# XuyangBai/PointDSC

Hardware: AMD Instinct MI355X
Metric: point-cloud pairs/sec @ N=5000 corr (higher is better)
Workload: dtype f32 (attention products as fp16x3 split (fp16 hi+lo operand pairs, three f16 MFMAs per product), f32 accumulate; fc_message / PointCN products as fp16 hi+lo split; spatial-consistency matrix stored as unorm16); 1 GPU; 3DMatch-like synthetic correspondences (BASELINE.json configs[2]): N=5000 corr, 32 pairs per step sharded over 1 GPU(s) = 32 per GPU, 12-layer PointDSC, seeded random weights; num_corr=5000, pairs_per_gpu=32, global_batch=32, compat_format=u16, layer_gemm=h3, att_leaves=canonical, latency_mode=False, range_guard=lazy (pipeline), collective=none (single process, no process group)

## Files before the change

include/pointdsc_hip.h:

```cpp
#ifndef POINTDSC_HIP_H
#define POINTDSC_HIP_H

#include <stddef.h>

#ifdef __cplusplus
extern "C" {
#endif

#define PDSC_VERSION 9
#define PDSC_CHANNELS 128
#define PDSC_MAX_K 64
#define PDSC_MAX_POWER_ITERS 32

enum pdsc_status {
    PDSC_OK = 0,
    PDSC_ERR_ARG = -1,
    PDSC_ERR_WORKSPACE = -2,
    PDSC_ERR_LAUNCH = -3
};

typedef struct pdsc_config {
    int in_dim;
    int num_layers;
    int num_channels;
// ... 145 lines not shown
int    pdsc_pack_qkv_split(const float* qkv, void* q_split, void* kv_tiles, int bs, int N, void* stream);
size_t pdsc_attention_split_scratch_bytes(int bs, int N, int nsplit);
int    pdsc_attention_split_default_split(int bs, int N);
int    pdsc_attention_leaf_count(int N);
int    pdsc_attention_leaf_plan(int bs, int N, int leaves_mode, int* nsplit, int* nleaf);
size_t pdsc_attention_leaf_scratch_bytes(int bs, int N, int leaves_mode);
int    pdsc_sc_attention_split(const void* q_split, const void* kv_tiles, const float* compat, long long ld,
                               float* msg, void* scratch, size_t scratch_bytes, int bs, int N, int nsplit,
                               void* stream);
int    pdsc_sc_attention_split_u16(const void* q_split, const void* kv_tiles, const unsigned short* compat_u16, long long ld,
                                   float* msg, void* scratch, size_t scratch_bytes, int bs, int N, int nsplit,
                                   void* stream);

int pdsc_attention_trace(long long* device_buffer);

int pdsc_layer_trace(long long* device_buffer);

int pdsc_classifier_hidden(const float* feat, const float* W1, const float* b1, const float* W2, const float* b2, float* h2,
                           int M, void* stream);

int pdsc_normalize_confidence(const float* feat, const float* h2, const float* w3, const float* b3,
                              float* normed, float* conf, int M, void* stream);

int pdsc_nms_keys(const float* src_keypts, const float* conf, float radius, float* keys,
                  int bs, int N, void* stream);
size_t pdsc_nms_workspace_bytes(int bs, int N);
int pdsc_nms_keys_grid(const float* src_keypts, const float* conf, float radius, float* keys, void* workspace,
                       size_t workspace_bytes, int bs, int N, void* stream);
int pdsc_rank_select(const float* keys, int* seeds, int bs, int N, int num_seeds, void* stream);

// ... 187 lines not shown
```

pointdsc_amd/_lib.py:

```python
from __future__ import annotations

import ctypes as C
import os
from pathlib import Path

PKG = Path(__file__).resolve().parent
LIB_PATH = Path(os.environ.get("POINTDSC_HIP_LIB", PKG / "libpointdsc_hip.so"))


class PointDSCLibraryError(RuntimeError):
    pass


class PdscConfig(C.Structure):
    _fields_ = [
        ("in_dim", C.c_int), ("num_layers", C.c_int), ("num_channels", C.c_int),
        ("num_iterations", C.c_int), ("k", C.c_int), ("refine_iters", C.c_int),
        ("inlier_threshold", C.c_float), ("nms_radius", C.c_float), ("refine_threshold", C.c_float),
        ("attention_precision", C.c_int), ("compat_format", C.c_int), ("layer_gemm", C.c_int),
        ("att_leaves", C.c_int), ("value_fold", C.c_int),
    ]


W_SECTIONS = [
# ... 40 lines not shown
    "pdsc_wfrag_head_bytes": (_sz, []),
    "pdsc_wfrag_fold_tail_bytes": (_sz, []),
    "pdsc_wfrag_fold_head_bytes": (_sz, []),
    "pdsc_wfrag_build_tail": (_i, [_vp] * 7 + [_i, _vp]),
    "pdsc_wfrag_build_head": (_i, [_vp] * 5 + [_i, _vp]),
    "pdsc_sc_attention_split_partials": (_i, [_vp, _vp, _vp, _i, _ll, _vp, _sz, _i, _i, _i, _i, _vp]),
    "pdsc_split_q_bytes": (_sz, [_i, _i]),
    "pdsc_split_kv_bytes": (_sz, [_i, _i]),
    "pdsc_pack_qkv_split": (_i, [_vp, _vp, _vp, _i, _i, _vp]),
    "pdsc_attention_split_scratch_bytes": (_sz, [_i, _i, _i]),
    "pdsc_attention_split_default_split": (_i, [_i, _i]),
    "pdsc_attention_leaf_count": (_i, [_i]),
    "pdsc_attention_leaf_plan": (_i, [_i, _i, _i, C.POINTER(C.c_int), C.POINTER(C.c_int)]),
    "pdsc_attention_leaf_scratch_bytes": (_sz, [_i, _i, _i]),
    "pdsc_attention_trace": (_i, [_vp]),
    "pdsc_layer_trace": (_i, [_vp]),
    "pdsc_sc_attention_split": (_i, [_vp, _vp, _vp, _ll, _vp, _vp, _sz, _i, _i, _i, _vp]),
    "pdsc_sc_attention_split_u16": (_i, [_vp, _vp, _vp, _ll, _vp, _vp, _sz, _i, _i, _i, _vp]),
    "pdsc_attention_scratch_bytes": (_sz, [_i, _i, _i]),
    "pdsc_attention_default_split": (_i, [_i, _i]),
    "pdsc_sc_attention": (_i, [_vp, _vp, _ll, _vp, _vp, _sz, _i, _i, _i, _vp]),
    "pdsc_normalize_confidence": (_i, [_vp, _vp, _vp, _vp, _vp, _vp, _i, _vp]),
    "pdsc_nms_keys": (_i, [_vp, _vp, _f, _vp, _i, _i, _vp]),
    "pdsc_nms_workspace_bytes": (_sz, [_i, _i]),
    "pdsc_nms_keys_grid": (_i, [_vp, _vp, _f, _vp, _vp, _sz, _i, _i, _vp]),
    "pdsc_rank_select": (_i, [_vp, _vp, _i, _i, _i, _vp]),
    "pdsc_knn_seeds": (_i, [_vp, _vp, _vp, _vp, _i, _i, _i, _i, _vp]),
    "pdsc_knn_seeds_form": (_i, [_vp, _vp, _vp, _vp, _vp, _i, _i, _i, _i, _i, _vp]),
    "pdsc_normalize_confidence_pf": (_i, [_vp, _vp, _vp, _vp, _vp, _vp, _vp, _i, _i, _vp]),
    "pdsc_seed_power_iteration": (_i, [_vp, _vp, _vp, _vp, _vp, _vp, _vp, _vp, _vp, _i, _i, _i, _i, _i, _vp]),
# ... 97 lines not shown
```

pointdsc_amd/csrc/api.hip:

```cpp
#include <stdarg.h>
#include <stdlib.h>
#include <string.h>
#include <mutex>
#include "pdsc_common.h"
#include "ragged.h"
#include "attention_common.h"
#include "layer_args.h"

namespace pdsc {

static thread_local char g_err[512] = "";

static unsigned int*& range_report_slot() {
    static thread_local unsigned int* slot = nullptr;
    return slot;
}

void set_error(const char* fmt, ...) {
    va_list ap;
    va_start(ap, fmt);
    vsnprintf(g_err, sizeof(g_err), fmt, ap);
    va_end(ap);
}

// ... 333 lines not shown
    do {                               \
        const int rc__ = (call);       \
        if (rc__ != PDSC_OK) return rc__; \
    } while (0)

struct EncoderPlan {
    bool fused;
    bool split;
    LayerKernel kernel;
    bool x3, frag;
    bool fuse_merge;
    bool pf, leaves, fold;
    int gemm;
    int ns, Npad;
    int nleaf, value_width;
    int ws_tail, ws_head;
};

static int plan_encoder(const pdsc_config* cfg, int bs, int N, const int* nvalid, int n_min, EncoderPlan* plan) {
    EncoderPlan& p = *plan = EncoderPlan{};
    p.split = cfg->attention_precision != PDSC_ATT_FP32;
    p.x3 = cfg->attention_precision == PDSC_ATT_FP16X3_ALL;
    p.fused = env_int("PDSC_FUSED_LAYERS", 1) != 0 && cfg->num_layers > 0;
    const bool canonical = cfg->att_leaves >= PDSC_LEAVES_CANONICAL;
    const int min_tiles = (n_min + 31) / 32;
    p.ns = p.split ? pdsc_attention_split_default_split(bs, N) : 0;
#define PDSC_REQUIRE_SHORTEST_PAIR(cond)                                                                                             \
    PDSC_REQUIRE(cond, "pdsc_forward_testing_ragged: the shortest pair (%d correspondences) has fewer 32-key tiles than the key split " \
                 "planned for bs=%d, N=%d (%d): batch pairs of more similar size", n_min, bs, N, p.ns)
    if (nvalid && p.split && !canonical) PDSC_REQUIRE_SHORTEST_PAIR(min_tiles >= p.ns);
// ... 5 lines not shown
    if (!p.fused || !p.split) {
        p.kernel = by_size(1, bs * N);
        return PDSC_OK;
    }
    p.Npad = (int)round_up(N, 256);
    p.gemm = env_int("PDSC_LAYER_GEMM", cfg->layer_gemm) == PDSC_LAYER_GEMM_H3 ? PDSC_LAYER_GEMM_H3 : PDSC_LAYER_GEMM_F32;
    const bool h3 = p.gemm == PDSC_LAYER_GEMM_H3;
    const LayerKernel natural = by_size(bs, N);
    p.frag = env_int("PDSC_LAYER_FRAG", 1) && !p.x3 && !force_block && (natural == LayerKernel::Wave || h3);
    p.kernel = p.x3     ? LayerKernel::X3
               : !p.frag ? natural
                         : h3 && env_int("PDSC_LAYER_H3_VARIANT", 1) != 0 ? LayerKernel::H3 : LayerKernel::Wave;
    p.fuse_merge = env_int("PDSC_FUSE_MERGE", 1) && p.ns > 1 && p.ns <= layer_merge_limit(p.kernel);
    const bool pf_ok = p.kernel == LayerKernel::H3 && env_int("PDSC_LAYER_PF", 1) != 0;
    int lf_ns = 0, lf_nw = 0;
    if (canonical) leaf_plan(bs, N, cfg->att_leaves, &lf_nw, &lf_ns, &p.nleaf);
    p.leaves = pf_ok && canonical && (!nvalid || min_tiles >= 2 * p.nleaf);
    if (nvalid && !p.leaves) PDSC_REQUIRE_SHORTEST_PAIR(min_tiles >= p.ns);
#undef PDSC_REQUIRE_SHORTEST_PAIR
    p.pf = p.leaves || (pf_ok && p.fuse_merge);
    p.fold = cfg->value_fold == PDSC_VALUE_FOLD_ON && p.pf && N <= PDSC_VALUE_FOLD_MAX_N;
    p.value_width = p.fold ? PDSC_CHANNELS / 2 : PDSC_CHANNELS;
    p.ws_tail = p.fold ? PDSC_WS_FOLD_TAIL_H3 : h3 ? PDSC_WS_FRAG_TAIL_H3 : PDSC_WS_FRAG_TAIL;
    p.ws_head = p.fold ? PDSC_WS_FOLD_HEAD_H3 : h3 ? PDSC_WS_FRAG_HEAD_H3 : PDSC_WS_FRAG_HEAD;
    return PDSC_OK;
}

enum class ForwardMode { Testing, Validation, Probe };

struct ForwardCall {
    ForwardMode mode;
// ... 86 lines not shown
    else
        PDSC_TRY(pdsc_spatial_compat(c.src, c.tgt, x.W(PDSC_W_SIGMA_SPAT, 0), x.compat, nullptr, x.ld, c.bs, c.N, x.st));
    PDSC_TRY(launch_layer0(c.corr_pos, c.cfg->in_dim, x.W(PDSC_W_LAYER0_W, 0), x.W(PDSC_W_LAYER0_B, 0), x.featA, x.M, x.range_flag, c.bs, x.st));
    return probe_absmax(x, PDSC_RANGE_LAYER0, x.featA, (size_t)x.M * PDSC_CHANNELS);
}

static int attention_split(const ForwardCtx& x, float* msg_out, int nsplit) {
    return launch_attention_split_ex(x.q_split, x.kv_tiles, x.compat, x.cfmt, x.ld, msg_out, x.att_scratch, x.L.bytes[WS_ATT_SCRATCH], x.c.bs,
                                     x.c.N, nsplit, PDSC_PARTIALS_ROWS, x.c.nvalid, x.st);
}

static int run_fused_layer(const ForwardCtx& x, int i, bool last, const float* cur, float* nxt) {
    const EncoderPlan& plan = x.plan;
    const bool tail = i >= 0, head = !last, split = x.split;
    const bool parts = plan.pf || plan.fuse_merge;
    const int nparts = plan.leaves ? plan.nleaf : plan.ns;
    const float* part_o = parts ? (const float*)x.att_scratch : nullptr;
    const float* part_ml = parts ? part_o + (size_t)x.c.bs * nparts * plan.Npad * plan.value_width : nullptr;
    pdsc_layer_call c{};
    c.bs = split ? x.c.bs : 1; c.N = split ? x.c.N : x.M;
    if (tail) {
        c.msg = parts ? nullptr : x.msg;
        c.part_o = part_o; c.part_ml = part_ml; c.nsplit = nparts; c.Npad = plan.Npad;
        c.res = cur;
    } else
        c.feat_in = x.featA;
    if (last) c.feat_out = x.featA;
    if (head) {
        c.featB_out = nxt; c.qkv_out = split ? nullptr : x.qkv;
        c.q_split = x.q_split; c.kv_tiles = x.kv_tiles;
    }
    if (plan.frag) {
        if (tail) c.wfrag_tail = x.WS(plan.ws_tail, i);
// ... 1 lines not shown
        c.gemm_format = plan.gemm;
    } else {
        auto mat = [&](int section, int l) { return plan.x3 ? x.WS(section, l) : (const void*)x.W(section, l); };
        if (tail) {
            c.w1 = mat(PDSC_W_FC1_W, i); c.b1 = x.W(PDSC_W_FC1_B, i); c.w2 = mat(PDSC_W_FC2_W, i); c.b2 = x.W(PDSC_W_FC2_B, i);
            c.w3 = mat(PDSC_W_FC3_W, i); c.b3 = x.W(PDSC_W_FC3_B, i);
        }
        if (head) {
            c.wp = mat(PDSC_W_PCN_W, i + 1); c.bp = x.W(PDSC_W_PCN_B, i + 1); c.wq = mat(PDSC_W_QKV_W, i + 1); c.bq = x.W(PDSC_W_QKV_B, i + 1);
            if (split) c.wq_split = x.WS(PDSC_W_QKV_W, i + 1);
        }
    }
    if (plan.pf) c.io_flags = (tail ? PDSC_IO_PARTIALS_PF | PDSC_IO_RES_PF : 0) | (head ? PDSC_IO_FEATB_PF : 0);
    LayerArgs a = layer_args_from_call(c);
    a.nvalid = split ? x.c.nvalid : nullptr;
    if (plan.pf) {
        a.value_fold = plan.fold;
        a.range_flag = x.range_flag;
    } else
        a.trace = pdsc_layer_trace_buffer();
    PDSC_TRY(validate_layer_args(a, plan.kernel, "pdsc_forward_testing(layer)"));
    return dispatch_layer(a, plan.kernel, x.st);
}

static int run_encoder_fused(const ForwardCtx& x) {
    const ForwardCall& c = x.c;
    const EncoderPlan& plan = x.plan;
    const size_t att_bytes = x.L.bytes[WS_ATT_SCRATCH];
    PDSC_TRY(run_fused_layer(x, -1, false, nullptr, x.featB));
    float *cur = x.featB, *nxt = x.featC;
// ... 190 lines not shown
```

pointdsc_amd/csrc/attention_split.hip:

```cpp
#include <stdlib.h>
#include <type_traits>
#include "attention_common.h"
#include "split_layout.h"
#include "ragged.h"

namespace pdsc {


template <int NW, int BYTES>
__device__ __forceinline__ void issue_linear(__amdgpu_buffer_rsrc_t rsrc, int src_off, unsigned char* dst, int wave, unsigned lane16) {
    constexpr int PIECES = BYTES / 1024;
    static_assert(BYTES % 1024 == 0, "tile parts are whole KiB");
#pragma unroll
    for (int u = 0; u < (PIECES + NW - 1) / NW; ++u) {
        const int i = wave + NW * u;
        if ((u + 1) * NW <= PIECES || i < PIECES)
            __builtin_amdgcn_raw_ptr_buffer_load_lds(rsrc, (lptr_t)(dst + i * 1024), 16, lane16, src_off + i * 1024, 0, 0);
    }
}
__device__ __forceinline__ f32x16 scale_acc(f32x16 o, float alpha) {
#pragma unroll
    for (int r = 0; r < 16; ++r) {
        float v = o[r];
        asm volatile("v_mul_f32 %0, %0, %1" : "+v"(v) : "v"(alpha));
// ... 138 lines not shown
        dma_k(kt0);
        if (kt0 + 1 < kt1) dma_k(kt0 + 1);
        dma_v(kt0);
        asm volatile("s_waitcnt vmcnt(0)" ::: "memory");
        __syncthreads();
        for (int kt = kt0; kt < kt1; ++kt) {
            const int st = (kt - kt0) & 1;
            asm volatile("s_waitcnt vmcnt(0)" ::: "memory");
            __syncthreads();
            if (kt + 1 < kt1) {
#pragma unroll
                for (int slot = NCS; slot < DMA_SLOTS; ++slot) dma_slot(kt, st, slot);
            }
        }
        asm volatile("s_waitcnt vmcnt(0)" ::: "memory");
        if (!(a.nsplit != 1 && a.part_frag)) __syncthreads();
        return;
    }

    f32x4 ccur[4], cnext[4];
    dma_k(kt0); dma_c(kt0);
    if (CREG) creg_load(kt0, ccur);
    if (kt0 + 1 < kt1) { dma_k(kt0 + 1); dma_c(kt0 + 1); }
    if (CREG) creg_load(kt0 + 1, cnext);
    dma_v(kt0);
    sp16x8 qh[8], ql[8];
    auto load_q = [&](int pair, int qblock) {
        const int qrow = min(qblock * (NW * 32) + wave * 32 + l31, N - 1);
        const sp16* qsrc = a.qs + ((size_t)pair * NS + qrow) * SPL_Q_LD + 8 * h;
#pragma unroll
        for (int j = 0; j < 8; ++j) {
// ... 28 lines not shown
        for (int c = 0; c < NC; ++c)
#pragma unroll
            for (int g = 0; g < 4; ++g)
                *reinterpret_cast<f32x4*>(base + pf_offset_floats(4 * c + g)) = f32x4{o[c][4 * g], o[c][4 * g + 1], o[c][4 * g + 2], o[c][4 * g + 3]};
        if (h == 0) {
            a.part_ml[(slot_prev + l31) * 2 + 0] = m_prev;
            a.part_ml[(slot_prev + l31) * 2 + 1] = l_prev;
        }
#pragma unroll
        for (int c = 0; c < NC; ++c)
#pragma unroll
            for (int r = 0; r < 16; ++r) o[c][r] = 0.f;
    };

    const int q0w = qb * (NW * 32) + wave * 32;
    auto leaf_store = [&](int lf, float m_st, float l_st) {
        const size_t slot = ((size_t)b * a.nleaf + lf) * a.Npad + q0w;
        float* base = a.part_o + slot * VW + lane * 4;
#pragma unroll
        for (int c = 0; c < NC; ++c)
#pragma unroll
            for (int g = 0; g < 4; ++g)
                *reinterpret_cast<f32x4*>(base + pf_offset_floats(4 * c + g)) = f32x4{o[c][4 * g], o[c][4 * g + 1], o[c][4 * g + 2], o[c][4 * g + 3]};
        if (h == 0) {
            a.part_ml[(slot + l31) * 2 + 0] = m_st;
            a.part_ml[(slot + l31) * 2 + 1] = l_st;
        }
    };
    int leaf_prev = 0;

    const int koff = l31 * 16 + 512 * h;
    const int voff = l31 * 16 + (VW * 16) * h;
    const int crow_off = (wave * 32 + l31) * CROW;
    const int csw = C16 ? (l31 >> 2) & 3 : ((wave * 32 + l31) >> 1) & 7;
    constexpr float C16_INV = 1.0f / 65535.0f;
    typedef float f32x2 __attribute__((ext_vector_type(2)));
    f32x2 c16_inv2 = {C16_INV, C16_INV};
    asm volatile("" : "+v"(c16_inv2));
    auto c16_group = [&](const unsigned (&w)[8], int g, float (&cc)[4]) {
        const unsigned w0 = w[2 * g], w1 = w[2 * g + 1];
        const f32x2 a = f32x2{(float)(w0 & 0xffffu), (float)(w0 >> 16)} * c16_inv2;
        const f32x2 b = f32x2{(float)(w1 & 0xffffu), (float)(w1 >> 16)} * c16_inv2;
// ... 286 lines not shown
        b = b_n; sp = sp_n; qb = qb_n;
        kt0 = kt0n;
        kt1 = kt0 + per + (sp < rem ? 1 : 0);
        q_rows = q_rows_n;
        dK = 2; dV = 1;
        load_q(b, qb);
        l_run = 0.f;
        look_ahead();
    }
  }
    asm volatile("s_waitcnt vmcnt(0)" ::: "memory");
    if constexpr (PS) return;
    const float l_tot = l_run + __shfl_xor(l_run, 32, 64);
    const int q0 = qb * (NW * 32) + wave * 32;
    if constexpr (MG) {
        leaf_store(leaf, m_run, l_tot);
        return;
    }
    if (a.nsplit != 1 && a.part_frag) {
        float* base = a.part_o + (((size_t)b * a.nsplit + sp) * a.Npad + q0) * VW + lane * 4;
#pragma unroll
        for (int c = 0; c < NC; ++c)
#pragma unroll
            for (int g = 0; g < 4; ++g)
                *reinterpret_cast<f32x4*>(base + pf_offset_floats(4 * c + g)) = f32x4{o[c][4 * g], o[c][4 * g + 1], o[c][4 * g + 2], o[c][4 * g + 3]};
        if (h == 0 && q0 + l31 < a.Npad) {
            const size_t slot = ((size_t)b * a.nsplit + sp) * a.Npad + q0 + l31;
            a.part_ml[slot * 2 + 0] = m_run;
            a.part_ml[slot * 2 + 1] = l_tot;
        }
        if (TRACE) {
// ... 115 lines not shown
        const int rounds = ceil_div(wgs, slots);
        double cost = (double)rounds * (ceil_div(tiles, ns) + (ns > 1 ? 4.0 : 3.0));
        if (((ns * bs) & 7) != 0) cost *= 1.03;
        if (cost < best_cost - 1e-9) { best_cost = cost; best = ns; }
    }
    const int force_nw = env_int("PDSC_ATT_SPLIT_NW", 0), force_ns = env_int("PDSC_ATT_SPLIT_NS", 0);
    *nw_out = (force_nw == 4 || force_nw == 8) ? force_nw : nw;
    *nsplit_out = force_ns > 0 ? (force_ns < tiles ? force_ns : tiles) : best;
}

int attention_leaf_count(int N) {
    const int t = spl_num_tiles(N);
    return t >= 48 ? 4 : t >= 32 ? 8 : t >= 16 ? 4 : t >= 8 ? 2 : 1;
}

void leaf_plan(int bs, int N, int leaves_mode, int* nw_out, int* nsplit_out, int* nleaf_out) {
    int nw, ns;
    split_plan(bs, N, &nw, &ns);
    const int tiles = spl_num_tiles(N);
    int C = leaves_mode == PDSC_LEAVES_CANONICAL ? attention_leaf_count(N) : leaves_mode;
    if (C > tiles / 2) C = tiles / 2;
    if (C > PDSC_ATT_MAX_LEAVES) C = PDSC_ATT_MAX_LEAVES;
    if (C < 1) C = 1;
    const int nq = ceil_div(N, nw * 32), slots = nw == 8 ? 256 : 512;
    int best = 1;
    double best_cost = 1e30;
    for (int d = 1; d <= C; ++d) {
        if (C % d) continue;
        const int wgs = nq * bs * d, rounds = ceil_div(wgs, slots);
        double cost = (double)rounds * (ceil_div(tiles, d) + 4.0 + 0.35 * (C / d));
        if (((d * bs) & 7) != 0) cost *= 1.03;
        if (cost < best_cost - 1e-9) { best_cost = cost; best = d; }
    }
    *nw_out = nw; *nsplit_out = best; *nleaf_out = C;
}

}

using namespace pdsc;

extern "C" int pdsc_attention_leaf_count(int N) { return N > 0 ? attention_leaf_count(N) : -1; }

extern "C" int pdsc_attention_leaf_plan(int bs, int N, int leaves_mode, int* nsplit, int* nleaf) {
    PDSC_REQUIRE(bs > 0 && N > 0 && leaves_mode >= PDSC_LEAVES_CANONICAL && leaves_mode <= PDSC_ATT_MAX_LEAVES && nsplit && nleaf,
                 "pdsc_attention_leaf_plan: bs=%d N=%d leaves_mode=%d", bs, N, leaves_mode);
    int nw;
    leaf_plan(bs, N, leaves_mode, &nw, nsplit, nleaf);
    return PDSC_OK;
}

extern "C" size_t pdsc_attention_leaf_scratch_bytes(int bs, int N, int leaves_mode) {
    if (bs <= 0 || N <= 0 || leaves_mode < PDSC_LEAVES_CANONICAL) return 0;
    int nw, ns, C;
    leaf_plan(bs, N, leaves_mode, &nw, &ns, &C);
    return (size_t)bs * C * round_up(N, 256) * (PDSC_CHANNELS + 2) * sizeof(float);
}

int pdsc::launch_attention_leaves(const void* q_split, const void* kv_tiles, const void* compat, int compat_format, long long ld,
                                  void* scratch, size_t scratch_bytes, int bs, int N, int leaves_mode, const int* nvalid, int n_min,
                                  hipStream_t st, int value_width) {
    PDSC_REQUIRE(q_split && kv_tiles && compat && scratch, "pdsc_sc_attention_leaves: null pointer");
    PDSC_REQUIRE(value_width == PDSC_CHANNELS || value_width == PDSC_CHANNELS / 2, "pdsc_sc_attention_leaves: value_width=%d", value_width);
    const bool v64 = value_width != PDSC_CHANNELS;
    PDSC_REQUIRE(bs > 0 && N > 0, "pdsc_sc_attention_leaves: bs=%d N=%d", bs, N);
    PDSC_REQUIRE(compat_format == PDSC_COMPAT_F32 || compat_format == PDSC_COMPAT_U16, "pdsc_sc_attention_leaves: compat_format=%d", compat_format);
    const bool c16 = compat_format == PDSC_COMPAT_U16;
    PDSC_REQUIRE(ld >= round_up(N, SPL_BK) && ld % (c16 ? 8 : 4) == 0,
                 "pdsc_sc_attention_leaves: ld=%lld must be a multiple of %d and >= N rounded up to 32", ld, c16 ? 8 : 4);
    int nw, ns, C;
    leaf_plan(bs, N, leaves_mode, &nw, &ns, &C);
    PDSC_REQUIRE(!nvalid || (n_min + 31) / 32 >= 2 * C, "pdsc_sc_attention_leaves: the shortest pair (%d correspondences) has fewer than two "
                 "32-key tiles for each of the %d leaves planned for bs=%d, N=%d", n_min, C, bs, N);
    const size_t need = (size_t)bs * C * round_up(N, 256) * (value_width + 2) * sizeof(float);
    if (scratch_bytes < need) {
        set_error("pdsc_sc_attention_leaves: scratch %zu < %zu bytes", scratch_bytes, need);
        return PDSC_ERR_WORKSPACE;
    }
    const int tiles = spl_num_tiles(N);
    AttSplitArgs a{};
    a.qs = (const sp16*)q_split; a.kv = (const unsigned char*)kv_tiles; a.compat = compat; a.ld = ld; a.msg = nullptr;
    a.N = N; a.Npad = (int)round_up(N, 256); a.nsplit = ns; a.num_tiles = tiles; a.bs = bs;
    a.nq = ceil_div(N, nw * 32);
    a.nleaf = C;
    a.part_o = (float*)scratch;
    a.part_ml = a.part_o + (size_t)bs * C * a.Npad * value_width;
// ... 222 lines not shown
```

pointdsc_amd/csrc/layer.hip:

```cpp
#include <stdlib.h>
#include <type_traits>
#include "pdsc_common.h"
#include "split_layout.h"
#include "merge_partials.h"
#include "layer_args.h"
#include "layer_block.h"

namespace pdsc {

constexpr int LF_ROWS = 32;
constexpr int LF_LD = PDSC_CHANNELS + 4;
constexpr int LF_TILE = LF_ROWS * LF_LD;


#define LF_STAMP(k)                                                                                   \
    if (a.trace && lane == 0) a.trace[(((size_t)blockIdx.y * gridDim.x + blockIdx.x) * 4 + wave) * 16 + (k)] = __builtin_readcyclecounter();

template <int K>
__device__ __forceinline__ void load_w(const float* __restrict__ W, int n0, int l31, int h, f32x4 (&w)[K / 8]) {
    const float* p = W + (size_t)(n0 + l31) * K + 4 * h;
#pragma unroll
    for (int q = 0; q < K / 8; ++q) w[q] = *reinterpret_cast<const f32x4*>(p + 8 * q);
}

// ... 276 lines not shown
    const bool frag = h3 || (kernel == LayerKernel::Wave && (a.wf_tail || a.wf_head));
    const int io = a.io_flags;
    PDSC_REQUIRE(tail || head, "%s: neither tail (msg / partials) nor head (featB_out) requested", who);
    PDSC_REQUIRE(a.bs > 0 && a.N > 0, "%s: bs=%d N=%d", who, a.bs, a.N);
    PDSC_REQUIRE(a.gemm_format == PDSC_LAYER_GEMM_F32 || a.gemm_format == PDSC_LAYER_GEMM_H3, "%s: gemm_format=%d", who, a.gemm_format);
    PDSC_REQUIRE((io & ~(PDSC_IO_PARTIALS_PF | PDSC_IO_RES_PF | PDSC_IO_FEATB_PF)) == 0, "%s: io_flags=%d", who, io);
    PDSC_REQUIRE(h3 || (io == 0 && !a.value_fold), "%s: point-fragment hand-offs and the folded layer exist in the H3 kernel only", who);
    PDSC_REQUIRE(!h3 || a.gemm_format == PDSC_LAYER_GEMM_H3, "%s: point-fragment hand-offs need gemm_format = PDSC_LAYER_GEMM_H3", who);
    PDSC_REQUIRE(!a.value_fold || (io & PDSC_IO_PARTIALS_PF) || !tail, "%s: the folded layer merges point-fragment partials", who);
    if (tail) {
        PDSC_REQUIRE(a.res && (frag ? a.wf_tail != nullptr : a.w1 && a.b1 && a.w2 && a.b2 && a.w3 && a.b3),
                     "%s: tail needs res and fc1..fc3 (natural layout or the tail stream)", who);
        if (!a.msg) PDSC_REQUIRE(a.part_ml && a.nsplit >= 1 && a.nsplit <= layer_merge_limit(kernel) && a.Npad >= a.N,
                                 "%s: partials need part_ml, 1 <= nsplit <= %d (what this launch's kernel merges), Npad >= N", who,
                                 layer_merge_limit(kernel));
        PDSC_REQUIRE(!(io & PDSC_IO_PARTIALS_PF) || (!a.msg && a.Npad % 32 == 0), "%s: PF partials come un-merged (msg NULL), Npad a multiple of 32", who);
    } else {
        PDSC_REQUIRE(a.feat_in, "%s: head-only needs feat_in", who);
        PDSC_REQUIRE(!(io & (PDSC_IO_PARTIALS_PF | PDSC_IO_RES_PF)), "%s: head-only takes feat_in in row order", who);
    }
    if (head) PDSC_REQUIRE((a.qkv_out || a.qs) && (frag ? a.wf_head != nullptr : a.wp && a.bp && a.wq && a.bq),
                           "%s: head needs qkv_out or the split streams, and pcn, qkv weights (natural layout or the head stream)", who);
    else PDSC_REQUIRE(a.feat_out && !(io & PDSC_IO_FEATB_PF), "%s: tail-only needs feat_out (row order)", who);
    PDSC_REQUIRE((a.qs == nullptr) == (a.kv == nullptr), "%s: q_split and kv_tiles go together", who);
    PDSC_REQUIRE(!h3 || launch_layer_h3_fits(a, tail, head), "%s: output set not served by the H3 kernel (head: the split streams "
                 "only; tail + head: no feat_out; tail only: feat_out)", who);
    return PDSC_OK;
}

int dispatch_layer(const LayerArgs& a, LayerKernel kernel, hipStream_t st) {
// ... 59 lines not shown
```

pointdsc_amd/csrc/layer_args.h:

```cpp
#pragma once
#include "pdsc_common.h"
#include "merge_partials.h"

namespace pdsc {

struct LayerArgs {
    const float* msg;
    const float* part_o;
    const float* part_ml;
    int nsplit, Npad;
    const float* res;
    const float* feat_in;
    float* feat_out;
    float* featB_out;
    float* qkv_out;
    const float *w1, *b1, *w2, *b2, *w3, *b3;
    const float *wp, *bp, *wq, *bq;
    const sp16* wq_split;
    sp16* qs;
    unsigned char* kv;
    int N, bs;
    const unsigned char* wf_tail;
    const unsigned char* wf_head;
    int gemm_format;
    int io_flags;
    int stagger_cycles, stagger_mode;
    long long* trace;
    unsigned int* range_flag;
    int value_fold;
    const int* nvalid;
};

enum class LayerKernel { Block, Wave, H3, X3 };
constexpr int layer_merge_limit(LayerKernel k) {
    return k == LayerKernel::Block ? MERGE_MAX_SPLIT_BLOCK : k == LayerKernel::H3 ? MERGE_MAX_SPLIT_H3 : MERGE_MAX_SPLIT;
}

inline LayerArgs layer_args_from_call(const pdsc_layer_call& c) {
    LayerArgs a{};
    a.msg = c.msg; a.part_o = c.part_o; a.part_ml = c.part_ml; a.nsplit = c.nsplit; a.Npad = c.Npad;
    a.res = c.res; a.feat_in = c.feat_in; a.feat_out = c.feat_out; a.featB_out = c.featB_out; a.qkv_out = c.qkv_out;
    a.qs = (sp16*)c.q_split; a.kv = (unsigned char*)c.kv_tiles;
    a.w1 = (const float*)c.w1; a.b1 = c.b1; a.w2 = (const float*)c.w2; a.b2 = c.b2; a.w3 = (const float*)c.w3; a.b3 = c.b3;
    a.wp = (const float*)c.wp; a.bp = c.bp; a.wq = (const float*)c.wq; a.bq = c.bq; a.wq_split = (const sp16*)c.wq_split;
    a.wf_tail = (const unsigned char*)c.wfrag_tail; a.wf_head = (const unsigned char*)c.wfrag_head;
    a.gemm_format = c.gemm_format; a.io_flags = c.io_flags;
    a.N = c.N; a.bs = c.bs;
    return a;
}

int validate_layer_args(const LayerArgs& a, LayerKernel kernel, const char* who);
int dispatch_layer(const LayerArgs& a, LayerKernel kernel, hipStream_t st);

int launch_layer_wave(const LayerArgs& a, bool tail, bool head, hipStream_t st);
int launch_layer_h3(const LayerArgs& a, bool tail, bool head, hipStream_t st);
// ... 13 lines not shown
```

pointdsc_amd/csrc/layer_coop.hip:

```cpp
#include <type_traits>
#include "pdsc_common.h"
#include "split_layout.h"
#include "merge_partials.h"
#include "layer_args.h"
#include "layer_wave.h"
#include "ragged.h"

namespace pdsc {

constexpr int LC_WAVES = 4;

struct CoopOps { u32x4 v[2][8][2][64]; };

template <bool QKV>
__device__ __forceinline__ void coop_finish(const f32x16& acc, const f32x16& cross, f32x4 (&v)[4]) {
#pragma unroll
    for (int g = 0; g < 4; ++g)
#pragma unroll
        for (int e = 0; e < 4; ++e) v[g][e] = QKV ? acc[4 * g + e] : fmaf(cross[4 * g + e], H3_INV, acc[4 * g + e]);
}

template <bool T, bool H, bool FB_PF, int NB, bool F = false>
__global__ __launch_bounds__(64 * LC_WAVES, NB <= 4 ? 2 : 1) void layer_h3_coop_kernel(LayerArgs a) {
    __shared__ __attribute__((aligned(16))) CoopOps ops;
// ... 44 lines not shown
    };
    using std::false_type; using std::true_type;
    auto put = [&](int set, int kk, const u32x4& oh, const u32x4& ol) { ops.v[set][kk][0][lane] = oh; ops.v[set][kk][1][lane] = ol; };
    f32x4 y3[4];
    f32x4 v[4];

    if constexpr (T) {
        f32x4 x0[4];
        if (F && !low) {
        } else if (a.msg) {
#pragma unroll
            for (int q = 0; q < 4; ++q) x0[q] = *reinterpret_cast<const f32x4*>(a.msg + row * VW + 8 * (4 * w + q) + 4 * h);
        } else {
            with_split_count<MERGE_MAX_SPLIT_H3>(a.nsplit, [&](auto ns_tag) {
                constexpr int NS = decltype(ns_tag)::value;
                const size_t slot0 = (size_t)b * NS * a.Npad + (row - (size_t)b * a.N);
                const MergeWeights<NS> mw = merge_row_weights<NS>(a.part_ml, slot0, (size_t)a.Npad);
                const bool pf = a.io_flags & PDSC_IO_PARTIALS_PF;
                const size_t e0 = pf ? ((size_t)b * NS * a.Npad + (size_t)td.tile * 32) * VW + lane * 4 : slot0 * VW + 4 * h;
                const int eq = pf ? 256 : 8;
                constexpr int GQ = NB > 4 ? 4 : NS <= 2 ? 4 : NS <= 4 ? 2 : 1;
#pragma unroll
                for (int q0 = 0; q0 < 4; q0 += GQ) {
                    f32x4 pv[GQ][NS];
#pragma unroll
                    for (int q = 0; q < GQ; ++q)
#pragma unroll
                        for (int sp = 0; sp < NS; ++sp) pv[q][sp] = *reinterpret_cast<const f32x4*>(a.part_o + e0 + (size_t)sp * a.Npad * VW + (size_t)eq * (4 * w + q0 + q));
#pragma unroll
                    for (int q = 0; q < GQ; ++q) {
#pragma unroll
                        for (int e = 0; e < 4; ++e) {
                            x0[q0 + q][e] = merge_apply<NS>(pv[q], mw, e);
                            if constexpr (GQ < 4) asm volatile("" : "+v"(x0[q0 + q][e]));
// ... 202 lines not shown
```

pointdsc_amd/csrc/layer_h3.hip:

```cpp
#include <stdlib.h>
#include <type_traits>
#include "pdsc_common.h"
#include "split_layout.h"
#include "merge_partials.h"
#include "layer_args.h"
#include "layer_wave.h"

namespace pdsc {

constexpr int PDSC_H3_COOP_TILES = 2560;

#define LH_STAMP(k) \
    if (TRACE && lane == 0) a.trace[(size_t)gw * 64 + (k)] = __builtin_readcyclecounter();

template <bool F = false>
constexpr int stage_tiles(int stage) { return stage == ST_FC1 || stage == ST_FC2 ? 2 : stage == ST_FC3 || stage == ST_PCN ? 4 : F ? 10 : 12; }

template <bool T, bool H, bool TRACE = false, int PIPE = 6, int EXP = 0, bool FB_PF = false, int NWV = LW_WAVES, int NBUF = 2, bool F = false>
__global__ __launch_bounds__(64 * NWV, NBUF > 2 ? 1 : 2) void layer_h3_kernel(LayerArgs a) {
    __shared__ __attribute__((aligned(16))) float Vs_all[NWV][32 * LW_VLD];
    const int lane = threadIdx.x & 63;
    const int wave = __builtin_amdgcn_readfirstlane(threadIdx.x >> 6);
    const int l31 = lane & 31, h = lane >> 5;
    const int tpp = ceil_div_dev(a.N, 32);
// ... 43 lines not shown
                }
                make_kstep<true>(x0[2 * kk], x0[2 * kk + 1], a1h[kk], a1l[kk], rmax);
            } else {
                make_kstep<true>(x0[2 * kk], x0[2 * kk + 1], a0h[kk], a0l[kk], rmax);
            }
        };
        if (a.msg) {
#pragma unroll
            for (int q = 0; q < NQ; ++q) x0[q] = *reinterpret_cast<const f32x4*>(a.msg + row * VW + 8 * q + 4 * h);
#pragma unroll
            for (int kk = 0; kk < NQ / 2; ++kk) first_operand(kk);
        } else {
            with_split_count<MERGE_MAX_SPLIT_H3>(a.nsplit, [&](auto ns_tag) {
                constexpr int NS = decltype(ns_tag)::value;
                constexpr int GQ = (NS <= 2 ? 16 : NS <= 4 ? 8 : 4) < NQ ? (NS <= 2 ? 16 : NS <= 4 ? 8 : 4) : NQ;
                const size_t slot0 = (size_t)b * NS * a.Npad + (row - (size_t)b * a.N);
                const bool pf = a.io_flags & PDSC_IO_PARTIALS_PF;
                const size_t e0 = pf ? ((size_t)b * NS * a.Npad + (size_t)tile * 32) * VW + lane * 4 : slot0 * VW + 4 * h;
                const int eq = pf ? 256 : 8;
                const MergeWeights<NS> mw = merge_row_weights<NS>(a.part_ml, slot0, (size_t)a.Npad);
#pragma unroll
                for (int q0 = 0; q0 < NQ; q0 += GQ) {
                    f32x4 pv[GQ][NS];
#pragma unroll
                    for (int q = 0; q < GQ; ++q)
#pragma unroll
                        for (int sp = 0; sp < NS; ++sp)
                            pv[q][sp] = (EXP & 4) ? f32x4{1.f, 2.f, 3.f, (float)lane}
                                                  : *reinterpret_cast<const f32x4*>(a.part_o + e0 + (size_t)sp * a.Npad * VW + eq * (q0 + q));
#pragma unroll
                    for (int q = 0; q < GQ; ++q) {
#pragma unroll
                        for (int e = 0; e < 4; ++e) {
// ... 287 lines not shown
```

pointdsc_amd/csrc/merge_partials.h:

```cpp
#pragma once
#include <type_traits>
#include "pdsc_common.h"

namespace pdsc {

constexpr int MERGE_MAX_SPLIT = 4;
constexpr int MERGE_MAX_SPLIT_BLOCK = 8;
constexpr int MERGE_MAX_SPLIT_H3 = 8;

template <int MAX, class F>
__device__ __forceinline__ void with_split_count(int ns, F&& f) {
    static_assert(MAX == 4 || MAX == 8, "the layer kernels merge up to 4 or up to 8 splits");
    using std::integral_constant;
    if constexpr (MAX == 4) {
        switch (ns) {
            case 1: f(integral_constant<int, 1>{}); break;
            case 2: f(integral_constant<int, 2>{}); break;
            case 3: f(integral_constant<int, 3>{}); break;
            default: f(integral_constant<int, 4>{}); break;
        }
    } else {
        switch (ns) {
            case 1: f(integral_constant<int, 1>{}); break;
            case 2: f(integral_constant<int, 2>{}); break;
            case 3: f(integral_constant<int, 3>{}); break;
            case 4: f(integral_constant<int, 4>{}); break;
            case 5: f(integral_constant<int, 5>{}); break;
            case 6: f(integral_constant<int, 6>{}); break;
            case 7: f(integral_constant<int, 7>{}); break;
            default: f(integral_constant<int, 8>{}); break;
        }
    }
}

template <int NS>
struct MergeWeights {
    float w[NS], rden;
};

template <int NS>
__device__ __forceinline__ MergeWeights<NS> merge_row_weights(const float* __restrict__ part_ml, size_t slot0, size_t sp_stride) {
    MergeWeights<NS> r;
    float ls[NS];
#pragma unroll
    for (int sp = 0; sp < NS; ++sp) {
        const float2 ml = *reinterpret_cast<const float2*>(part_ml + (slot0 + (size_t)sp * sp_stride) * 2);
        r.w[sp] = ml.x; ls[sp] = ml.y;
    }
    float mmax = r.w[0];
#pragma unroll
    for (int sp = 1; sp < NS; ++sp) mmax = fmaxf(mmax, r.w[sp]);
    float den = 0.f;
#pragma unroll
    for (int sp = 0; sp < NS; ++sp) {
        r.w[sp] = __builtin_amdgcn_exp2f(r.w[sp] - mmax);
        den = fmaf(ls[sp], r.w[sp], den);
    }
    r.rden = 1.0f / den;
    return r;
}

template <int NS>
__device__ __forceinline__ float merge_apply(const f32x4 (&pv)[NS], const MergeWeights<NS>& mw, int e) {
    float s = 0.f;
#pragma unroll
    for (int sp = 0; sp < NS; ++sp) s = fmaf(pv[sp][e], mw.w[sp], s);
    return s * mw.rden;
}
template <int NS>
__device__ __forceinline__ f32x4 merge_apply(const f32x4 (&pv)[NS], const MergeWeights<NS>& mw) {
    f32x4 v;
#pragma unroll
    for (int e = 0; e < 4; ++e) v[e] = merge_apply<NS>(pv, mw, e);
    return v;
}

}
```

pointdsc_amd/csrc/ragged.h:

```cpp
#pragma once
#include "pdsc_common.h"

namespace pdsc {

int launch_nms_keys_grid(const float* src, const float* conf, float radius, float* keys, void* workspace, size_t workspace_bytes,
                         int bs, int N, const int* nvalid, hipStream_t st);
int launch_rank_select(const float* keys, int* seeds, int bs, int N, int num_seeds, const int* nvalid, const int* svalid, hipStream_t st,
                       unsigned int* conv_mask_init = nullptr);
int launch_seed_solve_forward(const float* normed, const float* src, const float* tgt, const int* knn_idx, const float* sigma,
                              const float* sigma_spat, float* eig_iters, unsigned int* conv_mask, float* seed_trans, float* seed_weights,
                              int bs, int N, int S, int k, int num_iterations, bool mask_ready, hipStream_t st);
int launch_select_and_refine(const int* counts, const float* seed_trans, const float* src, const float* tgt, float inlier_threshold,
                             float refine_threshold, int max_iters, int* best, float* initial_trans, float* labels, float* final_trans,
                             int* solves, int bs, int N, int S, const int* nvalid, hipStream_t st, int* trace, const unsigned int* range_flag,
                             unsigned int* range_report = nullptr);
int launch_knn_seeds(const float* normed, const int* seeds, float* dist_scratch, int* knn_idx, int bs, int N, int S, int k,
                     const int* nvalid, hipStream_t st);
bool knn_seeds_uses_fused(int bs, int N, int S, int k);
int launch_knn_seeds_form(const float* normed, const float* normed_pf, const int* seeds, float* dist_scratch, int* knn_idx, int bs, int N,
                          int S, int k, const int* nvalid, int form, hipStream_t st);
int launch_normalize_conf_pf(const float* feat, const float* h2, const float* w3, const float* b3, float* normed, float* normed_pf,
                             float* conf, int bs, int N, hipStream_t st);
int launch_score_hypotheses_slp(const float* seed_trans, const float* src, const float* tgt, float thr2, int* counts, int bs, int N, int S,
                                const int* nvalid, hipStream_t st);
// ... 2 lines not shown
                            int N, int S, const int* nvalid, hipStream_t st);
int launch_select_best(const int* counts, const float* seed_trans, const float* src, const float* tgt, float inlier_threshold, int* best,
                       float* best_trans, float* labels, int bs, int N, int S, const int* nvalid, hipStream_t st);
int launch_post_refinement(const float* initial_trans, const float* src, const float* tgt, float threshold, int max_iters,
                           float* final_trans, int* solves, int bs, int N, const int* nvalid, hipStream_t st, int* trace = nullptr,
                           const unsigned int* range_flag = nullptr);
int launch_layer0(const float* corr_pos, int in_dim, const float* W0, const float* b0, float* feat, int M, unsigned int* range_flag, int bs,
                  hipStream_t st);
constexpr int PDSC_REFINE_TRACE = 24;
int launch_attention_split_ex(const void* q_split, const void* kv_tiles, const void* compat, int compat_format, long long ld,
                              float* msg, void* scratch, size_t scratch_bytes, int bs, int N, int nsplit, int partial_layout,
                              const int* nvalid, hipStream_t st, int value_width = PDSC_CHANNELS);

constexpr int PDSC_ATT_MAX_LEAVES = 8;
int attention_leaf_count(int N);
void leaf_plan(int bs, int N, int leaves_mode, int* nw_out, int* nsplit_out, int* nleaf_out);
int launch_attention_leaves(const void* q_split, const void* kv_tiles, const void* compat, int compat_format, long long ld,
                            void* scratch, size_t scratch_bytes, int bs, int N, int leaves_mode, const int* nvalid, int n_min,
                            hipStream_t st, int value_width = PDSC_CHANNELS);

}
```

Baseline: 2512 pairs/s.

## Merge attention leaves in-kernel when one workgroup covers all leaves

When the leaf plan picks a single split (one workgroup walks all key leaves sequentially), the attention kernel now merges the earlier leaf partials with its running state at the end and writes one pre-merged partial plus a combined normaliser. The planner is changed to prefer a split of one for 8-wave configs with enough query work. The layer kernel then sees a single partial, indexed through the new part_slots stride. This is meant to cut the partial-merge traffic and work in the following layer kernel, at the cost of less key-dimension parallelism in attention. A runtime override for the split count is also added.

```diff
diff --git a/include/pointdsc_hip.h b/include/pointdsc_hip.h
--- a/include/pointdsc_hip.h
+++ b/include/pointdsc_hip.h
@@ -183,6 +183,8 @@
 
 int pdsc_attention_trace(long long* device_buffer);
 
+int pdsc_attention_leaf_split_override(int d);
+
 int pdsc_layer_trace(long long* device_buffer);
 
 int pdsc_classifier_hidden(const float* feat, const float* W1, const float* b1, const float* W2, const float* b2, float* h2,
diff --git a/pointdsc_amd/_lib.py b/pointdsc_amd/_lib.py
--- a/pointdsc_amd/_lib.py
+++ b/pointdsc_amd/_lib.py
@@ -78,6 +78,7 @@
     "pdsc_attention_leaf_plan": (_i, [_i, _i, _i, C.POINTER(C.c_int), C.POINTER(C.c_int)]),
     "pdsc_attention_leaf_scratch_bytes": (_sz, [_i, _i, _i]),
     "pdsc_attention_trace": (_i, [_vp]),
+    "pdsc_attention_leaf_split_override": (_i, [_i]),
     "pdsc_layer_trace": (_i, [_vp]),
     "pdsc_sc_attention_split": (_i, [_vp, _vp, _vp, _ll, _vp, _vp, _sz, _i, _i, _i, _vp]),
     "pdsc_sc_attention_split_u16": (_i, [_vp, _vp, _vp, _ll, _vp, _vp, _sz, _i, _i, _i, _vp]),
diff --git a/pointdsc_amd/csrc/api.hip b/pointdsc_amd/csrc/api.hip
--- a/pointdsc_amd/csrc/api.hip
+++ b/pointdsc_amd/csrc/api.hip
@@ -371,6 +371,7 @@
     int gemm;
     int ns, Npad;
     int nleaf, value_width;
+    int leaf_ns;
     int ws_tail, ws_head;
 };
 
@@ -406,7 +407,8 @@
     p.fuse_merge = env_int("PDSC_FUSE_MERGE", 1) && p.ns > 1 && p.ns <= layer_merge_limit(p.kernel);
     const bool pf_ok = p.kernel == LayerKernel::H3 && env_int("PDSC_LAYER_PF", 1) != 0;
     int lf_ns = 0, lf_nw = 0;
-    if (canonical) leaf_plan(bs, N, cfg->att_leaves, &lf_nw, &lf_ns, &p.nleaf);
+    if (canonical) PDSC_TRY(leaf_plan(bs, N, cfg->att_leaves, &lf_nw, &lf_ns, &p.nleaf));
+    p.leaf_ns = lf_ns;
     p.leaves = pf_ok && canonical && (!nvalid || min_tiles >= 2 * p.nleaf);
     if (nvalid && !p.leaves) PDSC_REQUIRE_SHORTEST_PAIR(min_tiles >= p.ns);
 #undef PDSC_REQUIRE_SHORTEST_PAIR
@@ -523,9 +525,10 @@
     const EncoderPlan& plan = x.plan;
     const bool tail = i >= 0, head = !last, split = x.split;
     const bool parts = plan.pf || plan.fuse_merge;
-    const int nparts = plan.leaves ? plan.nleaf : plan.ns;
+    const int slots = plan.leaves ? plan.nleaf : plan.ns;
+    const int nparts = plan.leaves && plan.leaf_ns == 1 ? 1 : slots;
     const float* part_o = parts ? (const float*)x.att_scratch : nullptr;
-    const float* part_ml = parts ? part_o + (size_t)x.c.bs * nparts * plan.Npad * plan.value_width : nullptr;
+    const float* part_ml = parts ? part_o + (size_t)x.c.bs * slots * plan.Npad * plan.value_width : nullptr;
     pdsc_layer_call c{};
     c.bs = split ? x.c.bs : 1; c.N = split ? x.c.N : x.M;
     if (tail) {
@@ -557,6 +560,7 @@
     if (plan.pf) c.io_flags = (tail ? PDSC_IO_PARTIALS_PF | PDSC_IO_RES_PF : 0) | (head ? PDSC_IO_FEATB_PF : 0);
     LayerArgs a = layer_args_from_call(c);
     a.nvalid = split ? x.c.nvalid : nullptr;
+    if (tail) a.part_slots = slots;
     if (plan.pf) {
         a.value_fold = plan.fold;
         a.range_flag = x.range_flag;
diff --git a/pointdsc_amd/csrc/attention_split.hip b/pointdsc_amd/csrc/attention_split.hip
--- a/pointdsc_amd/csrc/attention_split.hip
+++ b/pointdsc_amd/csrc/attention_split.hip
@@ -1,6 +1,7 @@
 #include <stdlib.h>
 #include <type_traits>
 #include "attention_common.h"
+#include "merge_partials.h"
 #include "split_layout.h"
 #include "ragged.h"
 
@@ -176,7 +177,7 @@
             }
         }
         asm volatile("s_waitcnt vmcnt(0)" ::: "memory");
-        if (!(a.nsplit != 1 && a.part_frag)) __syncthreads();
+        if (!MG && !(a.nsplit != 1 && a.part_frag)) __syncthreads();
         return;
     }
 
@@ -235,6 +236,9 @@
     };
 
     const int q0w = qb * (NW * 32) + wave * 32;
+    auto leaf_store_ml = [&](size_t slot, float m_st, float l_st) {
+        *reinterpret_cast<float2*>(a.part_ml + (slot + l31) * 2) = float2{m_st, l_st};
+    };
     auto leaf_store = [&](int lf, float m_st, float l_st) {
         const size_t slot = ((size_t)b * a.nleaf + lf) * a.Npad + q0w;
         float* base = a.part_o + slot * VW + lane * 4;
@@ -243,10 +247,7 @@
 #pragma unroll
             for (int g = 0; g < 4; ++g)
                 *reinterpret_cast<f32x4*>(base + pf_offset_floats(4 * c + g)) = f32x4{o[c][4 * g], o[c][4 * g + 1], o[c][4 * g + 2], o[c][4 * g + 3]};
-        if (h == 0) {
-            a.part_ml[(slot + l31) * 2 + 0] = m_st;
-            a.part_ml[(slot + l31) * 2 + 1] = l_st;
-        }
+        leaf_store_ml(slot, m_st, l_st);
     };
     int leaf_prev = 0;
 
@@ -563,7 +564,44 @@
     const float l_tot = l_run + __shfl_xor(l_run, 32, 64);
     const int q0 = qb * (NW * 32) + wave * 32;
     if constexpr (MG) {
-        leaf_store(leaf, m_run, l_tot);
+        if (a.nsplit != 1 || a.nleaf == 1) {
+            leaf_store(leaf, m_run, l_tot);
+            return;
+        }
+        const size_t slot0 = (size_t)b * a.nleaf * a.Npad + q0w;
+        with_split_count<MERGE_MAX_SPLIT_H3>(a.nleaf, [&](auto nl_tag) {
+            constexpr int L = decltype(nl_tag)::value;
+            if constexpr (L >= 2) {
+                float2 ml[L];
+#pragma unroll
+                for (int lf = 0; lf < L - 1; ++lf) ml[lf] = *reinterpret_cast<const float2*>(a.part_ml + (slot0 + l31 + (size_t)lf * a.Npad) * 2);
+                ml[L - 1] = float2{m_run, l_tot};
+                float* base = a.part_o + slot0 * VW + lane * 4;
+                const size_t lstride = (size_t)a.Npad * VW;
+                constexpr int GQ = (L <= 4 ? 8 : 4) * 64 / VW;
+                MergeWeights<L> mw;
+#pragma unroll
+                for (int q0 = 0; q0 < 4 * NC; q0 += GQ) {
+                    f32x4 pv[GQ][L];
+#pragma unroll
+                    for (int q = 0; q < GQ; ++q)
+#pragma unroll
+                        for (int lf = 0; lf < L - 1; ++lf)
+                            pv[q][lf] = *reinterpret_cast<const f32x4*>(base + (size_t)lf * lstride + pf_offset_floats(q0 + q));
+                    if (q0 == 0) mw = merge_weights_of<L>(ml);
+#pragma unroll
+                    for (int q = 0; q < GQ; ++q) {
+                        const int c = (q0 + q) >> 2, g = (q0 + q) & 3;
+                        pv[q][L - 1] = f32x4{o[c][4 * g], o[c][4 * g + 1], o[c][4 * g + 2], o[c][4 * g + 3]};
+                        f32x4 v;
+#pragma unroll
+                        for (int e = 0; e < 4; ++e) v[e] = merge_chain<L>(pv[q], mw, e);
+                        *reinterpret_cast<f32x4*>(base + pf_offset_floats(q0 + q)) = v;
+                    }
+                }
+                leaf_store_ml(slot0, 0.f, mw.den);
+            }
+        });
         return;
     }
     if (a.nsplit != 1 && a.part_frag) {
@@ -709,7 +747,8 @@
     return t >= 48 ? 4 : t >= 32 ? 8 : t >= 16 ? 4 : t >= 8 ? 2 : 1;
 }
 
-void leaf_plan(int bs, int N, int leaves_mode, int* nw_out, int* nsplit_out, int* nleaf_out) {
+static int g_leaf_split_override = 0;
+int leaf_plan(int bs, int N, int leaves_mode, int* nw_out, int* nsplit_out, int* nleaf_out) {
     int nw, ns;
     split_plan(bs, N, &nw, &ns);
     const int tiles = spl_num_tiles(N);
@@ -727,7 +766,17 @@
         if (((d * bs) & 7) != 0) cost *= 1.03;
         if (cost < best_cost - 1e-9) { best_cost = cost; best = d; }
     }
+    if (C > 1 && nw == 8 && (long long)nq * bs >= slots) best = 1;
+    int force = g_leaf_split_override;
+#ifdef PDSC_EXPERIMENTS
+    if (force == 0) force = env_int("PDSC_ATT_LEAF_SPLIT", 0);
+#endif
     *nw_out = nw; *nsplit_out = best; *nleaf_out = C;
+    if (force != 0) {
+        PDSC_REQUIRE(force > 0 && C % force == 0, "attention leaf plan: the split override %d does not divide the %d leaves of N=%d", force, C, N);
+        *nsplit_out = force;
+    }
+    return PDSC_OK;
 }
 
 }
@@ -740,7 +789,12 @@
     PDSC_REQUIRE(bs > 0 && N > 0 && leaves_mode >= PDSC_LEAVES_CANONICAL && leaves_mode <= PDSC_ATT_MAX_LEAVES && nsplit && nleaf,
                  "pdsc_attention_leaf_plan: bs=%d N=%d leaves_mode=%d", bs, N, leaves_mode);
     int nw;
-    leaf_plan(bs, N, leaves_mode, &nw, nsplit, nleaf);
+    return leaf_plan(bs, N, leaves_mode, &nw, nsplit, nleaf);
+}
+
+extern "C" int pdsc_attention_leaf_split_override(int d) {
+    PDSC_REQUIRE(d >= 0 && d <= PDSC_ATT_MAX_LEAVES, "pdsc_attention_leaf_split_override: d=%d (0 = the planner decides, else a divisor of the leaf count)", d);
+    g_leaf_split_override = d;
     return PDSC_OK;
 }
 
@@ -763,7 +817,7 @@
     PDSC_REQUIRE(ld >= round_up(N, SPL_BK) && ld % (c16 ? 8 : 4) == 0,
                  "pdsc_sc_attention_leaves: ld=%lld must be a multiple of %d and >= N rounded up to 32", ld, c16 ? 8 : 4);
     int nw, ns, C;
-    leaf_plan(bs, N, leaves_mode, &nw, &ns, &C);
+    if (const int prc = leaf_plan(bs, N, leaves_mode, &nw, &ns, &C); prc != PDSC_OK) return prc;
     PDSC_REQUIRE(!nvalid || (n_min + 31) / 32 >= 2 * C, "pdsc_sc_attention_leaves: the shortest pair (%d correspondences) has fewer than two "
                  "32-key tiles for each of the %d leaves planned for bs=%d, N=%d", n_min, C, bs, N);
     const size_t need = (size_t)bs * C * round_up(N, 256) * (value_width + 2) * sizeof(float);
diff --git a/pointdsc_amd/csrc/layer.hip b/pointdsc_amd/csrc/layer.hip
--- a/pointdsc_amd/csrc/layer.hip
+++ b/pointdsc_amd/csrc/layer.hip
@@ -314,6 +314,9 @@
         if (!a.msg) PDSC_REQUIRE(a.part_ml && a.nsplit >= 1 && a.nsplit <= layer_merge_limit(kernel) && a.Npad >= a.N,
                                  "%s: partials need part_ml, 1 <= nsplit <= %d (what this launch's kernel merges), Npad >= N", who,
                                  layer_merge_limit(kernel));
+        if (!a.msg) PDSC_REQUIRE(a.part_slots == a.nsplit || (h3 && a.part_slots > a.nsplit),
+                                 "%s: part_slots=%d (partials per pair in the layout) must be nsplit=%d, or more in the H3 kernels", who,
+                                 a.part_slots, a.nsplit);
         PDSC_REQUIRE(!(io & PDSC_IO_PARTIALS_PF) || (!a.msg && a.Npad % 32 == 0), "%s: PF partials come un-merged (msg NULL), Npad a multiple of 32", who);
     } else {
         PDSC_REQUIRE(a.feat_in, "%s: head-only needs feat_in", who);
diff --git a/pointdsc_amd/csrc/layer_args.h b/pointdsc_amd/csrc/layer_args.h
--- a/pointdsc_amd/csrc/layer_args.h
+++ b/pointdsc_amd/csrc/layer_args.h
@@ -9,6 +9,7 @@
     const float* part_o;
     const float* part_ml;
     int nsplit, Npad;
+    int part_slots;
     const float* res;
     const float* feat_in;
     float* feat_out;
@@ -38,7 +39,7 @@
 
 inline LayerArgs layer_args_from_call(const pdsc_layer_call& c) {
     LayerArgs a{};
-    a.msg = c.msg; a.part_o = c.part_o; a.part_ml = c.part_ml; a.nsplit = c.nsplit; a.Npad = c.Npad;
+    a.msg = c.msg; a.part_o = c.part_o; a.part_ml = c.part_ml; a.nsplit = c.nsplit; a.part_slots = c.nsplit; a.Npad = c.Npad;
     a.res = c.res; a.feat_in = c.feat_in; a.feat_out = c.feat_out; a.featB_out = c.featB_out; a.qkv_out = c.qkv_out;
     a.qs = (sp16*)c.q_split; a.kv = (unsigned char*)c.kv_tiles;
     a.w1 = (const float*)c.w1; a.b1 = c.b1; a.w2 = (const float*)c.w2; a.b2 = c.b2; a.w3 = (const float*)c.w3; a.b3 = c.b3;
diff --git a/pointdsc_amd/csrc/layer_coop.hip b/pointdsc_amd/csrc/layer_coop.hip
--- a/pointdsc_amd/csrc/layer_coop.hip
+++ b/pointdsc_amd/csrc/layer_coop.hip
@@ -82,10 +82,10 @@
         } else {
             with_split_count<MERGE_MAX_SPLIT_H3>(a.nsplit, [&](auto ns_tag) {
                 constexpr int NS = decltype(ns_tag)::value;
-                const size_t slot0 = (size_t)b * NS * a.Npad + (row - (size_t)b * a.N);
+                const size_t slot0 = (size_t)b * a.part_slots * a.Npad + (row - (size_t)b * a.N);
                 const MergeWeights<NS> mw = merge_row_weights<NS>(a.part_ml, slot0, (size_t)a.Npad);
                 const bool pf = a.io_flags & PDSC_IO_PARTIALS_PF;
-                const size_t e0 = pf ? ((size_t)b * NS * a.Npad + (size_t)td.tile * 32) * VW + lane * 4 : slot0 * VW + 4 * h;
+                const size_t e0 = pf ? ((size_t)b * a.part_slots * a.Npad + (size_t)td.tile * 32) * VW + lane * 4 : slot0 * VW + 4 * h;
                 const int eq = pf ? 256 : 8;
                 constexpr int GQ = NB > 4 ? 4 : NS <= 2 ? 4 : NS <= 4 ? 2 : 1;
 #pragma unroll
diff --git a/pointdsc_amd/csrc/layer_h3.hip b/pointdsc_amd/csrc/layer_h3.hip
--- a/pointdsc_amd/csrc/layer_h3.hip
+++ b/pointdsc_amd/csrc/layer_h3.hip
@@ -81,9 +81,9 @@
             with_split_count<MERGE_MAX_SPLIT_H3>(a.nsplit, [&](auto ns_tag) {
                 constexpr int NS = decltype(ns_tag)::value;
                 constexpr int GQ = (NS <= 2 ? 16 : NS <= 4 ? 8 : 4) < NQ ? (NS <= 2 ? 16 : NS <= 4 ? 8 : 4) : NQ;
-                const size_t slot0 = (size_t)b * NS * a.Npad + (row - (size_t)b * a.N);
+                const size_t slot0 = (size_t)b * a.part_slots * a.Npad + (row - (size_t)b * a.N);
                 const bool pf = a.io_flags & PDSC_IO_PARTIALS_PF;
-                const size_t e0 = pf ? ((size_t)b * NS * a.Npad + (size_t)tile * 32) * VW + lane * 4 : slot0 * VW + 4 * h;
+                const size_t e0 = pf ? ((size_t)b * a.part_slots * a.Npad + (size_t)tile * 32) * VW + lane * 4 : slot0 * VW + 4 * h;
                 const int eq = pf ? 256 : 8;
                 const MergeWeights<NS> mw = merge_row_weights<NS>(a.part_ml, slot0, (size_t)a.Npad);
 #pragma unroll
diff --git a/pointdsc_amd/csrc/merge_partials.h b/pointdsc_amd/csrc/merge_partials.h
--- a/pointdsc_amd/csrc/merge_partials.h
+++ b/pointdsc_amd/csrc/merge_partials.h
@@ -35,18 +35,15 @@
 
 template <int NS>
 struct MergeWeights {
-    float w[NS], rden;
+    float w[NS], den, rden;
 };
 
 template <int NS>
-__device__ __forceinline__ MergeWeights<NS> merge_row_weights(const float* __restrict__ part_ml, size_t slot0, size_t sp_stride) {
+__device__ __forceinline__ MergeWeights<NS> merge_weights_of(const float2 (&ml)[NS]) {
     MergeWeights<NS> r;
     float ls[NS];
 #pragma unroll
-    for (int sp = 0; sp < NS; ++sp) {
-        const float2 ml = *reinterpret_cast<const float2*>(part_ml + (slot0 + (size_t)sp * sp_stride) * 2);
-        r.w[sp] = ml.x; ls[sp] = ml.y;
-    }
+    for (int sp = 0; sp < NS; ++sp) { r.w[sp] = ml[sp].x; ls[sp] = ml[sp].y; }
     float mmax = r.w[0];
 #pragma unroll
     for (int sp = 1; sp < NS; ++sp) mmax = fmaxf(mmax, r.w[sp]);
@@ -56,16 +53,28 @@
         r.w[sp] = __builtin_amdgcn_exp2f(r.w[sp] - mmax);
         den = fmaf(ls[sp], r.w[sp], den);
     }
+    r.den = den;
     r.rden = 1.0f / den;
     return r;
 }
+template <int NS>
+__device__ __forceinline__ MergeWeights<NS> merge_row_weights(const float* __restrict__ part_ml, size_t slot0, size_t sp_stride) {
+    float2 ml[NS];
+#pragma unroll
+    for (int sp = 0; sp < NS; ++sp) ml[sp] = *reinterpret_cast<const float2*>(part_ml + (slot0 + (size_t)sp * sp_stride) * 2);
+    return merge_weights_of<NS>(ml);
+}
 
 template <int NS>
-__device__ __forceinline__ float merge_apply(const f32x4 (&pv)[NS], const MergeWeights<NS>& mw, int e) {
+__device__ __forceinline__ float merge_chain(const f32x4 (&pv)[NS], const MergeWeights<NS>& mw, int e) {
     float s = 0.f;
 #pragma unroll
     for (int sp = 0; sp < NS; ++sp) s = fmaf(pv[sp][e], mw.w[sp], s);
-    return s * mw.rden;
+    return s;
+}
+template <int NS>
+__device__ __forceinline__ float merge_apply(const f32x4 (&pv)[NS], const MergeWeights<NS>& mw, int e) {
+    return merge_chain<NS>(pv, mw, e) * mw.rden;
 }
 template <int NS>
 __device__ __forceinline__ f32x4 merge_apply(const f32x4 (&pv)[NS], const MergeWeights<NS>& mw) {
diff --git a/pointdsc_amd/csrc/ragged.h b/pointdsc_amd/csrc/ragged.h
--- a/pointdsc_amd/csrc/ragged.h
+++ b/pointdsc_amd/csrc/ragged.h
@@ -40,7 +40,7 @@
 
 constexpr int PDSC_ATT_MAX_LEAVES = 8;
 int attention_leaf_count(int N);
-void leaf_plan(int bs, int N, int leaves_mode, int* nw_out, int* nsplit_out, int* nleaf_out);
+int leaf_plan(int bs, int N, int leaves_mode, int* nw_out, int* nsplit_out, int* nleaf_out);
 int launch_attention_leaves(const void* q_split, const void* kv_tiles, const void* compat, int compat_format, long long ld,
                             void* scratch, size_t scratch_bytes, int bs, int N, int leaves_mode, const int* nvalid, int n_min,
                             hipStream_t st, int value_width = PDSC_CHANNELS);
```

Result: faster. 2548 pairs/s, median of 6 (+1.5%).
